# jerinphilip/whisper.tflite

Measured on AMD Instinct MI355X. Metric: audio-sec/s (RTF) whisper-tiny 30s clips batch=32 at 1/2/4/8 MI355X, higher is better.
Workload: dtype f32 (operands as two fp16 planes, f16 MFMA, f32 accumulate); 1 GPU; whisper-tiny batch=32x30s synthetic mel U(-1,1.5), fp32, random-init weights (BASELINE.json configs[1]); mel resident in HBM -> token ids on host; clips_per_gpu=32, global_batch=32, decoder_positions=30, argmax_steps=27, parallelism=clip-parallel dp1, one RCCL all_gather of id records per 8 batches, pipelined=True, batches_in_flight=10, decoder=2 consecutive steps' batches share one decoder chain (dec_pair, dec_group), last_batches_announced=2, priming_batches=1

## Files before the change

include/wt_debug.h:

```cpp
#ifndef WT_DEBUG_H_
#define WT_DEBUG_H_
#include "wt_capi.h"
#ifdef __cplusplus
extern "C" {
#endif
int wt_dbg_gemm(wt_engine* h, int M, int N, int K, const float* A, const float* W, const float* bias,
                const float* R, const float* pos, int pos_period, int epi, float* C);
int wt_dbg_gemm_planes(wt_engine* h, int M, int N, int K, const float* A, const float* W, const float* bias,
                       const float* R, const float* pos, int pos_period, int epi, int planes_out, int iters, float* C,
                       float* avg_ms, int n_cu );
int wt_dbg_set_forced_ids(wt_engine* h, const int64_t* ids, int clips);
int wt_dbg_set_plane_gemm_mode(int mode);
int wt_dbg_gemm_planes_ln(wt_engine* h, int M, int K, const float* A, const float* W, const float* bias, const float* R,
                          const float* pos, int pos_period, int epi, const float* ln_g, const float* ln_b, int n_cu,
                          float* C, float* ln_out, float* ln_y32, int* fused);
int wt_dbg_encoder_attention_planes(wt_engine* h, int batch, int T, int heads, const float* qkv, int iters, float* out,
                                    float* avg_ms);
int wt_dbg_gemm_bench(wt_engine* h, int M, int N, int K, int epi, int variant, int iters, float* avg_ms);
int wt_dbg_interference(wt_engine* h, const float* d_mel, int batch, int n_enc, int chain_len, int blocks,
                        float* enc_ms, float* chain_ms);
int wt_dbg_concurrency(wt_engine* h, const float* d_mel, int batch, int n_dec, int n_enc, float* dec_ms,
                       float* enc_ms);
int wt_dbg_dec_gemm_bench(wt_engine* h, int kind, int B, int N, int K, int rows, int iters, float* avg_us);
int wt_dbg_dec_gemm(wt_engine* h, int mode, int B, int N, int K, const float* X, const float* W,
// ... 35 lines not shown
                               float* kcache, float* vcache, float* out);
int wt_dbg_cross_attention_bf16(wt_engine* h, int batch, int heads, int T, int chunks, int nq, const float* x,
                                const float* ln_g, const float* ln_b, const float* wq, const float* bq, const float* kc,
                                const float* vc, float* out);
int wt_dbg_beam_topk(wt_engine* h, int rows, int V, int ldl, int kk, const float* logits, float* m, float* s,
                     uint64_t* keys);
int wt_dbg_beam_step(wt_engine* h, int K, int clips, int c0, int n_live, int pos, int n_prompt, int V, int64_t eot,
                     const float* logits, const int64_t* ids, float* live_sum, int32_t* fin_tok, float* fin_sum,
                     int32_t* fin_len, int32_t* n_fin, int32_t* done, int32_t* parent, int64_t* token, int64_t* ids_next);
int wt_dbg_beam_reorder(wt_engine* h, int src_rows, int dst_rows, int cap, int d, int slabs, int pos, int V,
                        const float* kv_src, float* kv_dst, const int64_t* ids_src, int64_t* ids_dst,
                        const int32_t* parent, const int64_t* token);
int wt_dbg_beam_finalize(wt_engine* h, int K, int clips, int c0, int pos, int n_prompt, const int64_t* ids,
                         const float* live_sum, int32_t* fin_tok, float* fin_sum, int32_t* fin_len, int32_t* n_fin,
                         const int32_t* done, int64_t* out_ids, int32_t* out_n, float* out_sum, int32_t* out_len);
int wt_dbg_dec_gemm_ksplit(wt_engine* h, int bf16, int M, int B, int N, int K, const float* X, const float* W,
                           const float* bias, float* R, float* Y, float* part);
int wt_dbg_dec_ln_gemm_rows(wt_engine* h, int bf16, int M, int B, int N, int K, const float* xin, const float* xpart,
                            const int64_t* ids, int ids_stride, int pos, const float* tok_emb, const float* pos_emb,
                            int n_vocab, int n_pos, const float* ln_g, const float* ln_b, const float* W, const float* bias,
                            int gelu, float* Y, float* xout);
int wt_dbg_dec_logits(wt_engine* h, int bf16, int M, int V, int K, const float* xin, const float* xpart, const float* ln_g,
                      const float* ln_b, const float* E, int blocks, float* logits, uint64_t* records);
int wt_dbg_select_token(wt_engine* h, int B, int n_tiles, const uint64_t* records, int64_t* ids, int stride, int pos,
                        int32_t* n_ids, int32_t* finished, int64_t eot, int stop_at_eot, int keep_ids);
int wt_dbg_language_head(wt_engine* h, int rows, int d, int n_vocab, int lang_lo, int n_lang, int forced_lang, const float* x,
                         const float* xpart, const float* ln_g, const float* ln_b, const float* tok_emb, float* probs,
                         int32_t* lang, float* lang_prob, int64_t* ids, int ids_stride);
#ifdef __cplusplus
}
#endif
#endif
```

whisper.tflite_amd/__init__.py:

```python
from __future__ import annotations

import ctypes
import enum
import os
from ctypes import (POINTER, byref, c_char_p, c_float, c_int, c_int32, c_int64, c_long, c_size_t,
                    c_uint64, c_void_p)

import numpy as np

_HERE = os.path.dirname(os.path.abspath(__file__))
LIB_PATH = os.environ.get("WT_LIB_PATH") or os.path.join(_HERE, "lib", "libwhisper-tflite.so")

WT_OK = 0
WT_MAX_IDS = 32
WT_PIPELINE_DEPTH = 24
WT_LANGUAGE_AUTO = -1
CHUNK_SAMPLES = 480000
STATUS_NAMES = {0: "WT_OK", 1: "WT_ERR_INVALID_ARG", 2: "WT_ERR_IO", 3: "WT_ERR_FORMAT",
                4: "WT_ERR_UNSUPPORTED", 5: "WT_ERR_DEVICE", 6: "WT_ERR_BUFFER"}

CAPI_SYMBOLS = [
    "wt_device_alloc", "wt_device_free", "wt_device_upload", "wt_device_download", "wt_device_synchronize",
    "wt_engine_create", "wt_engine_destroy", "wt_last_error", "wt_engine_dims",
    "wt_engine_set_option", "wt_engine_get_option", "wt_engine_set_prompt", "wt_transcribe_pcm", "wt_transcribe_long_pcm", "wt_transcribe_file",
    "wt_logmel_batch", "wt_logmel_batch_dev", "wt_encdec_tokens_batch",
    "wt_encdec_tokens_batch_dev", "wt_transcribe_tokens_batch_dev", "wt_pipeline_submit_dev", "wt_pipeline_submit_pcm_dev", "wt_pipeline_collect",
    "wt_encdec_debug_batch",
    "wt_encdec_tokens_full_batch", "wt_encdec_tokens_full_batch_dev", "wt_transcribe_tokens_full_batch_dev",
    "wt_language_count", "wt_detect_language_batch", "wt_detect_language_batch_dev", "wt_detect_language_pcm", "wt_last_languages",
    "wt_last_timings", "wt_last_beam_scores", "wt_last_kernel_stats", "wt_decode_text", "wt_language_id", "wt_lang_code", "wt_wav_read_legacy",
    "wt_vocab_info", "wt_filters", "wt_write_synthetic_weights", "wt_write_synthetic_vocab",
    "wt_vocab_open", "wt_vocab_close", "wt_vocab_get_info", "wt_vocab_get_filters", "wt_vocab_size", "wt_vocab_token",
    "wt_vocab_decode", "wt_log_mel_spectrogram", "wt_convert_tflite", "wt_shutdown",
]
DEBUG_SYMBOLS = [
    "wt_dbg_cross_absorbed", "wt_dbg_cross_absorbed_bf16", "wt_dbg_gemm_planes_ln", "wt_dbg_gemm", "wt_dbg_gemm_bench", "wt_dbg_dec_gemm_bench", "wt_dbg_dec_gemm", "wt_dbg_dec_ln_gemm", "wt_dbg_layernorm", "wt_dbg_encoder_attention",
    "wt_dbg_cross_attention", "wt_dbg_self_attention", "wt_dbg_interference", "wt_dbg_concurrency",
    "wt_dbg_gemm_planes", "wt_dbg_set_plane_gemm_mode", "wt_dbg_set_forced_ids", "wt_dbg_dec_gemm_bf16", "wt_dbg_dec_ln_gemm_bf16",
    "wt_dbg_self_attention_bf16", "wt_dbg_cross_attention_bf16", "wt_dbg_encoder_attention_planes", "wt_dbg_gemm_bf16", "wt_dbg_gemm_bf16_ln", "wt_dbg_encoder_attention_bf16",
    "wt_dbg_beam_topk", "wt_dbg_beam_step", "wt_dbg_beam_reorder", "wt_dbg_beam_finalize",
    "wt_dbg_dec_gemm_ksplit", "wt_dbg_dec_ln_gemm_rows", "wt_dbg_dec_logits", "wt_dbg_select_token",
    "wt_dbg_cross_absorbed_chain", "wt_dbg_absorbed_query_matrix", "wt_dbg_language_head", "wt_dbg_self_attention_long",
]


class WtError(RuntimeError):
    def __init__(self, code: int, message: str):
        super().__init__(f"{STATUS_NAMES.get(code, code)}: {message}")
        self.code = code


class EngineType(enum.IntEnum):
    Monolith = 0
    EncDec = 1


class Dims(ctypes.Structure):
    _fields_ = [(n, c_int32) for n in (
        "n_mels", "n_audio_ctx", "n_audio_state", "n_audio_head", "n_audio_layer",
        "n_vocab", "n_text_ctx", "n_text_state", "n_text_head", "n_text_layer")]


class Timings(ctypes.Structure):
    _fields_ = [("logmel_ms", c_float), ("encoder_ms", c_float), ("cross_kv_ms", c_float),
# ... 87 lines not shown
        L.wt_device_upload.argtypes = [c_void_p, c_void_p, ctypes.c_size_t, c_void_p, ctypes.c_size_t]
        L.wt_device_download.argtypes = [c_void_p, c_void_p, c_void_p, ctypes.c_size_t, ctypes.c_size_t]
        L.wt_device_synchronize.argtypes = [c_void_p]
        L.wt_dbg_set_forced_ids.argtypes = [c_void_p, POINTER(c_int64), c_int]
        L.wt_dbg_dec_gemm_bf16.argtypes = L.wt_dbg_dec_gemm.argtypes
        L.wt_dbg_dec_ln_gemm_bf16.argtypes = L.wt_dbg_dec_ln_gemm.argtypes
        L.wt_dbg_encoder_attention.argtypes = [c_void_p, c_int, c_int, c_int, fp, fp]
        L.wt_dbg_cross_attention.argtypes = [c_void_p, c_int, c_int, c_int, c_int, c_int, fp, fp, fp, fp, fp, fp, fp, fp]
        L.wt_dbg_self_attention.argtypes = [c_void_p, c_int, c_int, c_int, c_int, c_int, fp, fp, fp, fp]
        L.wt_dbg_self_attention_bf16.argtypes = L.wt_dbg_self_attention.argtypes
        L.wt_dbg_cross_attention_bf16.argtypes = L.wt_dbg_cross_attention.argtypes
        u64p = POINTER(c_uint64)
        L.wt_dbg_beam_topk.argtypes = [c_void_p, c_int, c_int, c_int, c_int, fp, fp, fp, u64p]
        L.wt_dbg_beam_step.argtypes = [c_void_p, c_int, c_int, c_int, c_int, c_int, c_int, c_int, c_int64, fp, ip64, fp, ip32,
                                       fp, ip32, ip32, ip32, ip32, ip64, ip64]
        L.wt_dbg_beam_reorder.argtypes = [c_void_p, c_int, c_int, c_int, c_int, c_int, c_int, c_int, fp, fp, ip64, ip64, ip32,
                                          ip64]
        L.wt_dbg_beam_finalize.argtypes = [c_void_p, c_int, c_int, c_int, c_int, c_int, ip64, fp, ip32, fp, ip32, ip32, ip32,
                                           ip64, ip32, fp, ip32]
        L.wt_dbg_dec_gemm_ksplit.argtypes = [c_void_p, c_int, c_int, c_int, c_int, c_int, fp, fp, fp, fp, fp, fp]
        L.wt_dbg_dec_ln_gemm_rows.argtypes = [c_void_p, c_int, c_int, c_int, c_int, c_int, fp, fp, ip64, c_int, c_int, fp, fp,
                                              c_int, c_int, fp, fp, fp, fp, c_int, fp, fp]
        L.wt_dbg_dec_logits.argtypes = [c_void_p, c_int, c_int, c_int, c_int, fp, fp, fp, fp, fp, c_int, fp, u64p]
        L.wt_dbg_select_token.argtypes = [c_void_p, c_int, c_int, u64p, ip64, c_int, c_int, ip32, ip32, c_int64, c_int,
                                          c_int]
        L.wt_language_count.argtypes = [c_void_p]
        L.wt_detect_language_batch.argtypes = [c_void_p, fp, c_int, ip32, fp]
        L.wt_detect_language_batch_dev.argtypes = [c_void_p, c_void_p, c_int, ip32, fp]
        L.wt_detect_language_pcm.argtypes = [c_void_p, fp, c_size_t, ip32, fp]
        L.wt_last_languages.argtypes = [c_void_p, ip32, fp, c_int]
        L.wt_dbg_language_head.argtypes = [c_void_p, c_int, c_int, c_int, c_int, c_int, c_int, fp, fp, fp, fp, fp, fp, ip32, fp,
                                           ip64, c_int]
        L.wt_encdec_tokens_full_batch.argtypes = [c_void_p, fp, c_int, ip64, c_int, ip32]
        L.wt_encdec_tokens_full_batch_dev.argtypes = [c_void_p, c_void_p, c_int, ip64, c_int, ip32]
        L.wt_transcribe_tokens_full_batch_dev.argtypes = [c_void_p, c_void_p, c_int, ip64, c_int, ip32]
        L.wt_dbg_self_attention_long.argtypes = [c_void_p, c_int, c_int, c_int, c_int, fp, fp, fp, fp]
        _lib = L
    return _lib


def _f32(a) -> np.ndarray:
    return np.ascontiguousarray(a, dtype=np.float32)


def _fp(a: np.ndarray):
    return a.ctypes.data_as(POINTER(c_float)) if a is not None else None
# ... 635 lines not shown
        N, K = W.shape
        xin = _f32(xin) if xin is not None else None
        xpart = _f32(xpart) if xpart is not None else None
        ids_a = np.ascontiguousarray(ids, dtype=np.int64) if ids is not None else None
        tok_emb = _f32(tok_emb) if tok_emb is not None else None
        pos_emb = _f32(pos_emb) if pos_emb is not None else None
        if ids_a is not None:
            B, stride = ids_a.shape
            M = M or B
        else:
            M, stride = xin.shape[0], 0
            B = B or M
        xout = np.array(xout, np.float32, order="C") if xout is not None else np.zeros((M + 1, K), np.float32)
        assert xout.shape == (M + 1, K)
        Y = np.zeros((M, N), np.float32)
        self._check(lib().wt_dbg_dec_ln_gemm_rows(
            self._h, int(bf16), M, B, N, K, _fp(xin), _fp(xpart), _ip64(ids_a) if ids_a is not None else None, stride, pos,
            _fp(tok_emb), _fp(pos_emb), tok_emb.shape[0] if tok_emb is not None else 0,
            pos_emb.shape[0] if pos_emb is not None else 0, _fp(ln_g), _fp(ln_b), _fp(W), _fp(bias), int(gelu), _fp(Y),
            _fp(xout)))
        return Y, xout

    def dbg_dec_logits(self, xin, ln_g, ln_b, E, xpart=None, blocks=0, bf16=False, want_logits=True,
                       logits_guard=1.0e30, records_guard=0xA5A5A5A5A5A5A5A5):
        xin, ln_g, ln_b, E = _f32(xin), _f32(ln_g), _f32(ln_b), _f32(E)
        xpart = _f32(xpart) if xpart is not None else None
        M, K = xin.shape
        V = E.shape[0]
        logits = np.full((M + 1, V), logits_guard, np.float32) if want_logits else None
        records = np.full((M + 1, (V + 31) // 32), records_guard, np.uint64)
        self._check(lib().wt_dbg_dec_logits(self._h, int(bf16), M, V, K, _fp(xin), _fp(xpart), _fp(ln_g), _fp(ln_b), _fp(E),
                                            blocks, _fp(logits), records.ctypes.data_as(POINTER(c_uint64))))
        return logits, records

    def dbg_language_head(self, x, ln_g, ln_b, tok_emb, lang_lo, n_lang, xpart=None, ids=None, forced_lang=-1):
        x, ln_g, ln_b, tok_emb = _f32(x), _f32(ln_g), _f32(ln_b), _f32(tok_emb)
        xpart = _f32(xpart) if xpart is not None else None
        rows, d = x.shape
        probs = np.full((rows, n_lang), np.nan, np.float32)
        lang = np.full(rows, -1, np.int32)
        prob = np.full(rows, np.nan, np.float32)
        ids = np.array(ids, np.int64, order="C") if ids is not None else None
        self._check(lib().wt_dbg_language_head(
            self._h, rows, d, tok_emb.shape[0], lang_lo, n_lang, forced_lang, _fp(x), _fp(xpart), _fp(ln_g), _fp(ln_b),
            _fp(tok_emb), _fp(probs), _ip32(lang), _fp(prob), _ip64(ids) if ids is not None else None,
            ids.shape[1] if ids is not None else 0))
        return probs, lang, prob, ids

    def dbg_select_token(self, records, ids, pos, n_ids, finished, eot, stop_at_eot=True, keep_ids=False):
        records = np.ascontiguousarray(records, dtype=np.uint64)
        B, n_tiles = records.shape
        ids = np.array(ids, np.int64, order="C")
        n_ids = np.array(n_ids, np.int32, order="C")
        finished = np.array(finished, np.int32, order="C")
        self._check(lib().wt_dbg_select_token(self._h, B, n_tiles, records.ctypes.data_as(POINTER(c_uint64)), _ip64(ids),
# ... 38 lines not shown
```

whisper.tflite_amd/csrc/capi.cpp:

```cpp
#include "wt_capi.h"

#include <hip/hip_runtime.h>

#include <functional>

#include <cstdio>
#include <cstdlib>
#include <sys/stat.h>
#include <unistd.h>
#include <cmath>
#include <cstring>
#include <memory>
#include <string>
#include <vector>

#include <mutex>

#include "engine.h"
#include "tflite_extract.h"
#include "weights_gen.h"
#include "wt_debug.h"
#include "kernels.h"

struct wt_engine {
// ... 1773 lines not shown
    const size_t mk = size_t(M) * K;
    DevArr<float> dxin(xin ? mk : 0, xin), dxp(xpart ? mk : 0, xpart);
    DevArr<long long> dids(ids ? size_t(B) * ids_stride : 0, reinterpret_cast<const long long*>(ids));
    DevArr<float> dtok(ids ? size_t(n_vocab) * K : 0, tok_emb), dpos(ids ? size_t(n_pos) * K : 0, pos_emb);
    DevArr<float> dg(K, ln_g), db(K, ln_b), dB(N, bias), dY(size_t(M) * N);
    DevArr<float> dxo(mk + K, xout);
    wt::DecGemmArgs g;
    g.bf16 = bf;
    g.Wt = dW.w(); g.w_scale = dW.scale; g.N = N; g.K = K; g.B = B; g.M = M;
    g.ln_g = dg.p; g.ln_b = db.p; g.xout = dxo.p;
    if (ids) {
      g.ids = dids.p; g.ids_stride = ids_stride; g.pos = pos; g.tok_emb = dtok.p; g.pos_emb = dpos.p; g.n_vocab = n_vocab;
    } else {
      g.xin = dxin.p; g.xpart = xpart ? dxp.p : nullptr;
    }
    g.bias = dB.p; g.Y = dY.p; g.ldy = N;
    wt::launch_dec_gemm(g, wt::kProLn, gelu ? wt::kDecBiasGelu : wt::kDecBias, h->impl->stream());
    h->impl->sync();
    dY.to_host(Y);
    dxo.to_host(xout);
  });
}

int wt_dbg_dec_logits(wt_engine* h, int bf16, int M, int V, int K, const float* xin, const float* xpart, const float* ln_g,
                      const float* ln_b, const float* E, int blocks, float* logits, uint64_t* records) {
  if (!h || !xin || !ln_g || !ln_b || !E || !records || M < 1 || M > 128 || V < 1 || blocks < 0 ||
      (K != 128 && K != 384 && K != 512)) {
    return WT_ERR_INVALID_ARG;
  }
  return guarded(h, [&] {
    const bool bf = bf16 != 0;
    const int n_tiles = (V + 31) / 32;
    const DevTiled dE(E, V, K, bf);
    const size_t mk = size_t(M) * K;
    DevArr<float> dxin(mk, xin), dxp(xpart ? mk : 0, xpart), dg(K, ln_g), db(K, ln_b);
    DevArr<float> dY(logits ? (size_t(M) + 1) * V : 0, logits);
    DevArr<unsigned long long> dBest((size_t(M) + 1) * n_tiles, reinterpret_cast<const unsigned long long*>(records));
    wt::DecGemmArgs g;
    g.bf16 = bf;
    g.logits_blocks = blocks;
    g.Wt = dE.w(); g.w_scale = dE.scale; g.N = V; g.K = K; g.B = M; g.M = M;
    g.xin = dxin.p; g.xpart = xpart ? dxp.p : nullptr; g.ln_g = dg.p; g.ln_b = db.p;
    g.Y = logits ? dY.p : nullptr; g.ldy = V; g.best = dBest.p;
    wt::launch_dec_gemm(g, wt::kProLn, wt::kDecLogits, h->impl->stream());
    h->impl->sync();
    if (logits) dY.to_host(logits);
    dBest.to_host(reinterpret_cast<unsigned long long*>(records));
  });
}

int wt_dbg_select_token(wt_engine* h, int B, int n_tiles, const uint64_t* records, int64_t* ids, int stride, int pos,
                        int32_t* n_ids, int32_t* finished, int64_t eot, int stop_at_eot, int keep_ids) {
  if (!h || !records || !ids || !n_ids || !finished || B < 1 || n_tiles < 1 || pos < 0 || pos + 1 >= stride) {
    return WT_ERR_INVALID_ARG;
  }
  return guarded(h, [&] {
    DevArr<unsigned long long> dRec(size_t(B) * n_tiles, reinterpret_cast<const unsigned long long*>(records));
    DevArr<long long> dids(size_t(B) * stride, reinterpret_cast<const long long*>(ids));
    DevArr<int> dn(B, n_ids), dfin(B, finished);
    wt::launch_select_token(dRec.p, n_tiles, dids.p, stride, pos, dn.p, dfin.p, eot, stop_at_eot, B, h->impl->stream(),
                            keep_ids != 0);
    h->impl->sync();
    dids.to_host(reinterpret_cast<long long*>(ids));
    dn.to_host(n_ids);
    dfin.to_host(finished);
  });
}

int wt_dbg_language_head(wt_engine* h, int rows, int d, int n_vocab, int lang_lo, int n_lang, int forced_lang, const float* x,
                         const float* xpart, const float* ln_g, const float* ln_b, const float* tok_emb, float* probs,
                         int32_t* lang, float* lang_prob, int64_t* ids, int ids_stride) {
// ... 106 lines not shown
```

whisper.tflite_amd/csrc/k_decoder.hip:

```cpp
#include <hip/hip_runtime.h>

#include <cstdlib>

#include "bf16_split.h"
#include "kernels.h"

namespace wt {
namespace {

using f32x16 = __attribute__((ext_vector_type(16))) float;
using f32x4 = __attribute__((ext_vector_type(4))) float;
using half8 = __attribute__((ext_vector_type(8))) _Float16;

__device__ __forceinline__ float gelu_erf(float x) {
  return 0.5f * x * (1.0f + erff(x * 0.70710678118654752440f));
}
__device__ __forceinline__ unsigned ordered_bits(float v) {
  v = v + 0.0f;
  const unsigned u = __float_as_uint(v);
  return (u & 0x80000000u) ? ~u : (u | 0x80000000u);
}
__device__ __forceinline__ int crow(int r, int h) { return (r & 3) + 8 * (r >> 2) + 4 * h; }

struct DecGemmDev {
// ... 309 lines not shown
      const int m = (g0 + t) * 32 + crow(r, lh);
      float v = sum + bias;
      if (EPI == kDecBias && g.gelu) v = gelu_erf(v);
      const bool ok = n_ok && m < M;
      if (EPI == kDecResid && khalf == 1) {
        if (ok) g.part[(long)m * g.ldy + n_epi] = sum;
        continue;
      }
      if (EPI == kDecResid && ok) v += r_pre[EPI == kDecResid ? j : 0];
      if (ok && g.Y) g.Y[(long)m * g.ldy + n_epi] = v;
      if (EPI == kDecLogits) {
        unsigned long long p = ok ? (((unsigned long long)ordered_bits(v) << 32) | (unsigned)n_epi) : 0ull;
#pragma unroll
        for (int off = 16; off >= 1; off >>= 1) {
          const unsigned long long o2 = __shfl_xor(p, off, 64);
          p = o2 > p ? o2 : p;
        }
        if (l31 == 0 && m < M) g.best[(long)m * g.best_stride + tile] = p;
      }
    }
  }
}

template <int KS, bool BF, int LNMODE>
__global__ __launch_bounds__(256, 2) void dec_logits_persistent(DecGemmDev g) {
  constexpr int KC = KS * 64, XLD = KC + 4;
  constexpr int kRed = 2 * 4 * 16 * 64, kXs = LNMODE >= 0 ? 32 * XLD : 0;
  __shared__ __attribute__((aligned(16))) float smem_l[kRed > kXs ? kRed : kXs];
  float (*red)[4][16][64] = reinterpret_cast<float (*)[4][16][64]>(smem_l);
  const int tid = threadIdx.x, lane = tid & 63, wid = tid >> 6;
  const int l31 = lane & 31, lh = lane >> 5;
  const int n_tiles = (g.N + 31) / 32, K = g.K, M = g.M;
  const int k0 = wid * (K >> 2);
  constexpr int WSTEP = BF ? 512 : 1024;
  const unsigned short* const wbase = g.Wt + (long)(k0 >> 4) * WSTEP + lane * 8;
  const long tile_stride = (long)(K >> 4) * WSTEP;
  int tile = blockIdx.x;
  u32x4_t wh[KS], wl[BF ? 1 : KS];
  {
    const unsigned short* wp = wbase + (long)(tile < n_tiles ? tile : n_tiles - 1) * tile_stride;
#pragma unroll
    for (int s = 0; s < KS; ++s) {
      wh[s] = *reinterpret_cast<const u32x4_t*>(wp + (long)s * WSTEP);
      if (!BF) wl[s] = *reinterpret_cast<const u32x4_t*>(wp + (long)s * WSTEP + 512);
    }
  }
  u32x4_t ah[KS], al[BF ? 1 : KS];
  float inv = 1.0f;
  const int m0 = blockIdx.y * 32;
  if (LNMODE >= 0) {
    constexpr int NF4 = 2 * KS;
    const int r8 = lane >> 3, sub = lane & 7, lrow = wid * 8 + r8, row = m0 + lrow;
    const RowSrc src{g.xin, g.xpart, nullptr, 0, 0, g.B, nullptr, nullptr, 0};
    f32x4 v[NF4], gg[NF4], bb[NF4];
#pragma unroll
    for (int j = 0; j < NF4; ++j) {
      gg[j] = *reinterpret_cast<const f32x4*>(g.ln_g + (sub + 8 * j) * 4);
      bb[j] = *reinterpret_cast<const f32x4*>(g.ln_b + (sub + 8 * j) * 4);
    }
    load_row<NF4, LNMODE < 0 ? 0 : LNMODE>(v, src, row < M ? row : M - 1, sub, K);
    float mean, rstd;
    row_stats<NF4>(v, K, &mean, &rstd);
#pragma unroll
    for (int j = 0; j < NF4; ++j) {
      const int c = (sub + 8 * j) * 4;
      f32x4 o;
#pragma unroll
      for (int e = 0; e < 4; ++e) o[e] = (v[j][e] - mean) * rstd * gg[j][e] + bb[j][e];
      *reinterpret_cast<f32x4*>(&smem_l[lrow * XLD + c]) = o;
    }
    __syncthreads();
  }
  {
    int row = m0 + l31;
    row = row < M ? row : M - 1;
    const float* xp = (LNMODE >= 0 ? smem_l + l31 * XLD : g.X + (long)row * g.ldx) + k0 + 8 * lh;
    float xa[KS][8];
#pragma unroll
    for (int s = 0; s < KS; ++s) {
      const f32x4 a = *reinterpret_cast<const f32x4*>(xp + 16 * s);
      const f32x4 b = *reinterpret_cast<const f32x4*>(xp + 16 * s + 4);
#pragma unroll
      for (int e = 0; e < 4; ++e) {
        xa[s][e] = a[e];
        xa[s][4 + e] = b[e];
      }
    }
    if (BF) {
#pragma unroll
      for (int s = 0; s < KS; ++s)
#pragma unroll
        for (int e = 0; e < 4; ++e) ah[s][e] = pack_bf16x2(xa[s][2 * e], xa[s][2 * e + 1]);
    } else {
      float mx = 0.0f;
#pragma unroll
      for (int s = 0; s < KS; ++s)
#pragma unroll
        for (int e = 0; e < 8; ++e) mx = fmaxf(mx, fabsf(xa[s][e]));
      mx = fmaxf(mx, __shfl_xor(mx, 32, 64));
      const unsigned ex = (__float_as_uint(mx) >> 23) & 0xFFu;
      const float sc = ex < 32u ? 1.0f : __uint_as_float((268u - ex) << 23);
      inv = ex < 32u ? 1.0f : __uint_as_float((ex - 14u) << 23);
#pragma unroll
      for (int s = 0; s < KS; ++s) {
        u32x4_t pl[3];
        split8_f16x2(xa[s], sc, pl);
        ah[s] = pl[0];
        al[s] = pl[1];
      }
    }
  }
  if (LNMODE >= 0) __syncthreads();
  float rscale[16];
#pragma unroll
  for (int r = 0; r < 16; ++r) rscale[r] = BF ? 1.0f : __shfl(inv, crow(r, lh), 64) * g.w_descale;

  for (int par = 0; tile < n_tiles; tile += gridDim.x, par ^= 1) {
    const int nt = tile + (int)gridDim.x < n_tiles ? tile + (int)gridDim.x : tile;
    const unsigned short* np = wbase + (long)nt * tile_stride;
    u32x4_t nwh[KS], nwl[BF ? 1 : KS];
#pragma unroll
    for (int s = 0; s < KS; ++s) {
      nwh[s] = *reinterpret_cast<const u32x4_t*>(np + (long)s * WSTEP);
      if (!BF) nwl[s] = *reinterpret_cast<const u32x4_t*>(np + (long)s * WSTEP + 512);
    }
    f32x16 part;
#pragma unroll
    for (int r = 0; r < 16; ++r) part[r] = 0.0f;
#pragma unroll
    for (int s = 0; s < KS; ++s) {
      if (BF) {
        using bf16x8 = __attribute__((ext_vector_type(8))) __bf16;
        part = __builtin_amdgcn_mfma_f32_32x32x16_bf16(__builtin_bit_cast(bf16x8, ah[s]), __builtin_bit_cast(bf16x8, wh[s]), part, 0, 0, 0);
      } else {
        const half8 a_h = __builtin_bit_cast(half8, ah[s]), a_l = __builtin_bit_cast(half8, al[BF ? 0 : s]);
        const half8 b_h = __builtin_bit_cast(half8, wh[s]), b_l = __builtin_bit_cast(half8, wl[BF ? 0 : s]);
        part = __builtin_amdgcn_mfma_f32_32x32x16_f16(a_h, b_l, part, 0, 0, 0);
        part = __builtin_amdgcn_mfma_f32_32x32x16_f16(a_l, b_h, part, 0, 0, 0);
        part = __builtin_amdgcn_mfma_f32_32x32x16_f16(a_h, b_h, part, 0, 0, 0);
      }
    }
#pragma unroll
    for (int r = 0; r < 16; ++r) red[par][wid][r][lane] = BF ? part[r] : 0.0f + part[r] * rscale[r];
    __syncthreads();
    {
      const int n_epi = tile * 32 + l31;
      const bool n_ok = n_epi < g.N;
#pragma unroll
      for (int rr = 0; rr < 4; ++rr) {
        const int r = wid * 4 + rr;
        float v = red[par][0][r][lane];
        v += red[par][1][r][lane];
        v += red[par][2][r][lane];
        v += red[par][3][r][lane];
        v += 0.0f;
        const int m = m0 + crow(r, lh);
        const bool ok = n_ok && m < M;
        if (ok && g.Y) g.Y[(long)m * g.ldy + n_epi] = v;
        const unsigned key = ok ? ordered_bits(v) : 0u;
        unsigned kmax = key;
#pragma unroll
        for (int off = 16; off >= 1; off >>= 1) {
          const unsigned o2 = __shfl_xor(kmax, off, 64);
          kmax = o2 > kmax ? o2 : kmax;
        }
        const unsigned long long hit = __ballot(ok && key == kmax);
        const unsigned half_hits = (unsigned)(hit >> (32 * lh));
        if (l31 == 0 && m < M) {
          const unsigned col = half_hits ? (unsigned)(tile * 32 + 31 - __clz(half_hits)) : 0u;
          g.best[(long)m * g.best_stride + tile] = half_hits ? (((unsigned long long)kmax << 32) | col) : 0ull;
        }
      }
    }
#pragma unroll
    for (int s = 0; s < KS; ++s) {
      wh[s] = nwh[s];
      if (!BF) wl[s] = nwl[s];
    }
  }
}

template <bool BF, int LNMODE>
bool launch_logits_persistent(const DecGemmDev& g, hipStream_t s, int blocks = 0) {
  if (g.K % 64 != 0 || g.ksplit != 1) return false;
  const int n_tiles = (g.N + 31) / 32, m_tiles = (g.M + 31) / 32;
  static const int forced = [] {
    const char* v = getenv("WT_LOGITS_BLOCKS");
    const int n = v ? atoi(v) : 0;
    return n >= 32 && n <= 1024 ? n : 0;
  }();
  const int total = forced ? forced : (blocks >= 32 && blocks <= 1024 ? blocks : 512);
  const int per = total / m_tiles;
  const dim3 grid(n_tiles < per ? n_tiles : per, m_tiles);
  switch (g.K / 64) {
    case 2: hipLaunchKernelGGL((dec_logits_persistent<2, BF, LNMODE>), grid, dim3(256), 0, s, g); return true;
    case 6: hipLaunchKernelGGL((dec_logits_persistent<6, BF, LNMODE>), grid, dim3(256), 0, s, g); return true;
    case 8: hipLaunchKernelGGL((dec_logits_persistent<8, BF, LNMODE>), grid, dim3(256), 0, s, g); return true;
    default: return false;
  }
}

template <int NF4, int LNMODE>
__global__ __launch_bounds__(256) void dec_finalize_ln(RowSrc src, const float* __restrict__ g,
                                                       const float* __restrict__ b,
                                                       float* __restrict__ y, int B, int K) {
  const int lane = threadIdx.x & 63, wid = threadIdx.x >> 6;
  const int r8 = lane >> 3, sub = lane & 7;
  const int row = blockIdx.x * 32 + wid * 8 + r8;
  if (row >= B) return;
  f32x4 v[NF4], gg[NF4], bb[NF4];
#pragma unroll
  for (int j = 0; j < NF4; ++j) {
    gg[j] = *reinterpret_cast<const f32x4*>(g + (sub + 8 * j) * 4);
    bb[j] = *reinterpret_cast<const f32x4*>(b + (sub + 8 * j) * 4);
  }
  load_row<NF4, LNMODE>(v, src, row, sub, K);
  float mean, rstd;
  row_stats<NF4>(v, K, &mean, &rstd);
#pragma unroll
  for (int j = 0; j < NF4; ++j) {
// ... 39 lines not shown
  if (two) {
    launch_steps<PRO, EPI, NF4, LNMODE, WAVES, CH, 2, BF>(g, s);
  } else {
    launch_steps<PRO, EPI, NF4, LNMODE, WAVES, CH, 1, BF>(g, s);
  }
}

template <int LNMODE, bool BF>
void launch_ln(const DecGemmDev& g, hipStream_t s) {
  switch (g.K) {
    case 128: launch_gt<kProLn, kDecBias, 4, LNMODE, 4, 1, BF>(g, s); break;
    case 384: launch_gt<kProLn, kDecBias, 12, LNMODE, 4, 1, BF>(g, s); break;
    case 512: launch_gt<kProLn, kDecBias, 16, LNMODE, 4, 1, BF>(g, s); break;
    default: throw Error(kErrFormat, "decoder kernels support d_model 128, 384 or 512");
  }
}

}

template <bool BF>
static void dispatch_dec_gemm(const DecGemmArgs& a, const DecGemmDev& g, int pro, int epi, hipStream_t s) {
  if (pro == kProLn && epi == kDecLogits) {
    if (a.ids || !a.xin || !a.ln_g || !a.ln_b) throw Error(kErrInvalidArg, "logits GEMM: LayerNorm rows come from xin (+ xpart)");
    const bool ok = a.xpart ? launch_logits_persistent<BF, 3>(g, s, a.logits_blocks) : launch_logits_persistent<BF, 0>(g, s, a.logits_blocks);
    if (!ok) throw Error(kErrInvalidArg, "logits GEMM with the LayerNorm prologue: K must be a multiple of 64");
    return;
  }
  if (pro == kProLn) {
    if (epi != kDecBias) throw Error(kErrInvalidArg, "decoder GEMM: the LayerNorm prologue pairs with the bias epilogue");
    if (a.ids) {
      if (a.xpart) throw Error(kErrInvalidArg, "decoder GEMM: embedding rows have no pending partial");
      launch_ln<2, BF>(g, s);
    } else if (a.xpart) {
      launch_ln<3, BF>(g, s);
    } else {
      launch_ln<0, BF>(g, s);
    }
    return;
  }
  const int key = pro * 8 + epi;
  switch (key) {
    case kProNone * 8 + kDecResid: launch_gt<kProNone, kDecResid, 0, 0, 8, 1, BF>(g, s); break;
    case kProNone * 8 + kDecBias: launch_gt<kProNone, kDecBias, 0, 0, 4, 1, BF>(g, s); break;
    case kProNone * 8 + kDecLogits:
      if (!launch_logits_persistent<BF, -1>(g, s, a.logits_blocks)) launch_gt<kProNone, kDecLogits, 0, 0, 4, 1, BF>(g, s);
      break;
    case kProCombine * 8 + kDecResid:
      switch (a.chunks) {
        case 1: launch_gt<kProCombine, kDecResid, 0, 0, 8, 1, BF>(g, s); break;
        case 2: launch_gt<kProCombine, kDecResid, 0, 0, 8, 2, BF>(g, s); break;
        case 4: launch_gt<kProCombine, kDecResid, 0, 0, 8, 4, BF>(g, s); break;
        case 8: launch_gt<kProCombine, kDecResid, 0, 0, 8, 8, BF>(g, s); break;
        default: throw Error(kErrInvalidArg, "cross_chunks must be 1, 2, 4 or 8");
      }
      break;
    default: throw Error(kErrInvalidArg, "unsupported decoder GEMM prologue / epilogue pair");
  }
}

void launch_dec_gemm(const DecGemmArgs& a, int pro, int epi, hipStream_t s) {
  const int gelu = epi == kDecBiasGelu ? 1 : 0;
  if (epi == kDecBiasGelu) epi = kDecBias;
  const int M = a.M > 0 ? a.M : a.B;
  const int ksplit = a.ksplit > 0 ? a.ksplit : 1;
  DecGemmDev g{a.Wt,      1.0f / a.w_scale, a.N,  a.K,       M,         a.B,     a.X,     a.ldx,   a.xin,  a.xout,
               a.ln_g,    a.ln_b,    a.ids,      a.ids_stride, a.pos,   a.tok_emb, a.pos_emb, a.n_vocab,
               a.cross_ws, a.heads,  a.chunks,   a.bias,    gelu,      a.R,     a.Y,     a.ldy,   a.best,
               a.best_stride > 0 ? a.best_stride : (a.N + 31) / 32, ksplit, a.part,  a.xpart, 0};
// ... 42 lines not shown
```

whisper.tflite_amd/csrc/kernels.h:

```cpp
#pragma once
#include <hip/hip_runtime.h>
#include <hip/hip_ext.h>

#include <cstdint>
#include <vector>

#include "error.h"

namespace wt {

struct LaunchTimer {
  hipEvent_t start = nullptr, stop = nullptr;
};
extern thread_local LaunchTimer g_launch_timer;

#define WT_LAUNCH_TIMED(kernel, grid, block, smem, stream, ...)                                                      \
  do {                                                                                                                \
    if (::wt::g_launch_timer.start) {                                                                                 \
      hipExtLaunchKernelGGL(kernel, grid, block, smem, stream, ::wt::g_launch_timer.start, ::wt::g_launch_timer.stop, \
                            0, __VA_ARGS__);                                                                          \
    } else {                                                                                                          \
      hipLaunchKernelGGL(kernel, grid, block, smem, stream, __VA_ARGS__);                                             \
    }                                                                                                                 \
  } while (0)
// ... 61 lines not shown
  float* ln_y32 = nullptr;
  int* nonfinite = nullptr;
};
bool launch_gemm_planes(const PlaneGemmArgs& a, int epi, hipStream_t s);
int plane_gemm_mode();
void set_plane_gemm_mode(int m);
bool launch_gemm_bf16_planes(const PlaneGemmArgs& a, int epi, hipStream_t s);
std::vector<unsigned short> round_weights_bf16(const float* W, int N, int K, int Kpad);
std::vector<unsigned short> split_weight_planes(const float* W, int N, int K, int Kpad, float scale);

enum DecPro : int {
  kProNone = 0,
  kProLn = 1,
  kProCombine = 2
};
enum DecEpi : int {
  kDecResid = 0,
  kDecBias = 1,
  kDecBiasGelu = 2,
  kDecLogits = 3
};
struct DecGemmArgs {
  int logits_blocks = 0;
  const unsigned short* Wt = nullptr;
  float w_scale = 1.0f;
  int N = 0, K = 0, B = 0;
  int M = 0;
  const float* X = nullptr;
  int ldx = 0;
  const float* xin = nullptr;
  float* xout = nullptr;
  const float* ln_g = nullptr;
  const float* ln_b = nullptr;
  const long long* ids = nullptr;
  int ids_stride = 0, pos = 0;
  const float* tok_emb = nullptr;
  const float* pos_emb = nullptr;
  int n_vocab = 0;
  const float* cross_ws = nullptr;
  int heads = 0, chunks = 0;
  const float* bias = nullptr;
  const float* R = nullptr;
  float* Y = nullptr;
  int ldy = 0;
  unsigned long long* best = nullptr;
  int best_stride = 0;
// ... 147 lines not shown
```

Before: 150,000 audio-sec/s.

## Process two row tiles per block in persistent logits GEMM to reuse weight loads

The persistent decoder logits kernel can now handle two 32-row M tiles per block, so each vocab weight tile loaded from memory feeds two MFMA row tiles instead of one. This halves weight streaming over the large embedding matrix when M is at least 64. A compile-time option to prefetch two tiles ahead is also added but defaults to one. In exchange the kernel uses more registers and shared memory, and launch bounds drop to one block per SIMD occupancy hint, which may reduce latency hiding.

```diff
diff --git a/include/wt_debug.h b/include/wt_debug.h
--- a/include/wt_debug.h
+++ b/include/wt_debug.h
@@ -81,6 +81,8 @@
                             int gelu, float* Y, float* xout);
 int wt_dbg_dec_logits(wt_engine* h, int bf16, int M, int V, int K, const float* xin, const float* xpart, const float* ln_g,
                       const float* ln_b, const float* E, int blocks, float* logits, uint64_t* records);
+int wt_dbg_dec_logits_ex(wt_engine* h, int bf16, int M, int V, int K, const float* xin, const float* xpart, const float* ln_g,
+                         const float* ln_b, const float* E, int blocks, int row_tiles, float* logits, uint64_t* records);
 int wt_dbg_select_token(wt_engine* h, int B, int n_tiles, const uint64_t* records, int64_t* ids, int stride, int pos,
                         int32_t* n_ids, int32_t* finished, int64_t eot, int stop_at_eot, int keep_ids);
 int wt_dbg_language_head(wt_engine* h, int rows, int d, int n_vocab, int lang_lo, int n_lang, int forced_lang, const float* x,
diff --git a/whisper.tflite_amd/__init__.py b/whisper.tflite_amd/__init__.py
--- a/whisper.tflite_amd/__init__.py
+++ b/whisper.tflite_amd/__init__.py
@@ -39,7 +39,7 @@
     "wt_dbg_gemm_planes", "wt_dbg_set_plane_gemm_mode", "wt_dbg_set_forced_ids", "wt_dbg_dec_gemm_bf16", "wt_dbg_dec_ln_gemm_bf16",
     "wt_dbg_self_attention_bf16", "wt_dbg_cross_attention_bf16", "wt_dbg_encoder_attention_planes", "wt_dbg_gemm_bf16", "wt_dbg_gemm_bf16_ln", "wt_dbg_encoder_attention_bf16",
     "wt_dbg_beam_topk", "wt_dbg_beam_step", "wt_dbg_beam_reorder", "wt_dbg_beam_finalize",
-    "wt_dbg_dec_gemm_ksplit", "wt_dbg_dec_ln_gemm_rows", "wt_dbg_dec_logits", "wt_dbg_select_token",
+    "wt_dbg_dec_gemm_ksplit", "wt_dbg_dec_ln_gemm_rows", "wt_dbg_dec_logits", "wt_dbg_dec_logits_ex", "wt_dbg_select_token",
     "wt_dbg_cross_absorbed_chain", "wt_dbg_absorbed_query_matrix", "wt_dbg_language_head", "wt_dbg_self_attention_long",
 ]
 
@@ -173,6 +173,7 @@
         L.wt_dbg_dec_ln_gemm_rows.argtypes = [c_void_p, c_int, c_int, c_int, c_int, c_int, fp, fp, ip64, c_int, c_int, fp, fp,
                                               c_int, c_int, fp, fp, fp, fp, c_int, fp, fp]
         L.wt_dbg_dec_logits.argtypes = [c_void_p, c_int, c_int, c_int, c_int, fp, fp, fp, fp, fp, c_int, fp, u64p]
+        L.wt_dbg_dec_logits_ex.argtypes = [c_void_p, c_int, c_int, c_int, c_int, fp, fp, fp, fp, fp, c_int, c_int, fp, u64p]
         L.wt_dbg_select_token.argtypes = [c_void_p, c_int, c_int, u64p, ip64, c_int, c_int, ip32, ip32, c_int64, c_int,
                                           c_int]
         L.wt_language_count.argtypes = [c_void_p]
@@ -854,15 +855,16 @@
         return Y, xout
 
     def dbg_dec_logits(self, xin, ln_g, ln_b, E, xpart=None, blocks=0, bf16=False, want_logits=True,
-                       logits_guard=1.0e30, records_guard=0xA5A5A5A5A5A5A5A5):
-        xin, ln_g, ln_b, E = _f32(xin), _f32(ln_g), _f32(ln_b), _f32(E)
+                       logits_guard=1.0e30, records_guard=0xA5A5A5A5A5A5A5A5, row_tiles=0):
+        xin, E = _f32(xin), _f32(E)
+        ln_g, ln_b = (_f32(ln_g), _f32(ln_b)) if ln_g is not None else (None, None)
         xpart = _f32(xpart) if xpart is not None else None
         M, K = xin.shape
         V = E.shape[0]
         logits = np.full((M + 1, V), logits_guard, np.float32) if want_logits else None
         records = np.full((M + 1, (V + 31) // 32), records_guard, np.uint64)
-        self._check(lib().wt_dbg_dec_logits(self._h, int(bf16), M, V, K, _fp(xin), _fp(xpart), _fp(ln_g), _fp(ln_b), _fp(E),
-                                            blocks, _fp(logits), records.ctypes.data_as(POINTER(c_uint64))))
+        self._check(lib().wt_dbg_dec_logits_ex(self._h, int(bf16), M, V, K, _fp(xin), _fp(xpart), _fp(ln_g), _fp(ln_b), _fp(E),
+                                               blocks, row_tiles, _fp(logits), records.ctypes.data_as(POINTER(c_uint64))))
         return logits, records
 
     def dbg_language_head(self, x, ln_g, ln_b, tok_emb, lang_lo, n_lang, xpart=None, ids=None, forced_lang=-1):
diff --git a/whisper.tflite_amd/csrc/capi.cpp b/whisper.tflite_amd/csrc/capi.cpp
--- a/whisper.tflite_amd/csrc/capi.cpp
+++ b/whisper.tflite_amd/csrc/capi.cpp
@@ -1819,10 +1819,11 @@
   });
 }
 
-int wt_dbg_dec_logits(wt_engine* h, int bf16, int M, int V, int K, const float* xin, const float* xpart, const float* ln_g,
-                      const float* ln_b, const float* E, int blocks, float* logits, uint64_t* records) {
-  if (!h || !xin || !ln_g || !ln_b || !E || !records || M < 1 || M > 128 || V < 1 || blocks < 0 ||
-      (K != 128 && K != 384 && K != 512)) {
+int wt_dbg_dec_logits_ex(wt_engine* h, int bf16, int M, int V, int K, const float* xin, const float* xpart, const float* ln_g,
+                         const float* ln_b, const float* E, int blocks, int row_tiles, float* logits, uint64_t* records) {
+  const bool ln = ln_g && ln_b;
+  if (!h || !xin || (!ln && (ln_g || ln_b || xpart)) || !E || !records || M < 1 || M > 128 || V < 1 || blocks < 0 ||
+      row_tiles < 0 || row_tiles > 1 || (K != 128 && K != 384 && K != 512)) {
     return WT_ERR_INVALID_ARG;
   }
   return guarded(h, [&] {
@@ -1830,20 +1831,31 @@
     const int n_tiles = (V + 31) / 32;
     const DevTiled dE(E, V, K, bf);
     const size_t mk = size_t(M) * K;
-    DevArr<float> dxin(mk, xin), dxp(xpart ? mk : 0, xpart), dg(K, ln_g), db(K, ln_b);
+    DevArr<float> dxin(mk, xin), dxp(xpart ? mk : 0, xpart), dg(ln ? K : 0, ln_g), db(ln ? K : 0, ln_b);
     DevArr<float> dY(logits ? (size_t(M) + 1) * V : 0, logits);
     DevArr<unsigned long long> dBest((size_t(M) + 1) * n_tiles, reinterpret_cast<const unsigned long long*>(records));
     wt::DecGemmArgs g;
     g.bf16 = bf;
     g.logits_blocks = blocks;
+    g.logits_row_tiles = row_tiles;
     g.Wt = dE.w(); g.w_scale = dE.scale; g.N = V; g.K = K; g.B = M; g.M = M;
-    g.xin = dxin.p; g.xpart = xpart ? dxp.p : nullptr; g.ln_g = dg.p; g.ln_b = db.p;
+    if (ln) {
+      g.xin = dxin.p; g.xpart = xpart ? dxp.p : nullptr; g.ln_g = dg.p; g.ln_b = db.p;
+    } else {
+      g.X = dxin.p; g.ldx = K;
+    }
     g.Y = logits ? dY.p : nullptr; g.ldy = V; g.best = dBest.p;
-    wt::launch_dec_gemm(g, wt::kProLn, wt::kDecLogits, h->impl->stream());
+    wt::launch_dec_gemm(g, ln ? wt::kProLn : wt::kProNone, wt::kDecLogits, h->impl->stream());
     h->impl->sync();
     if (logits) dY.to_host(logits);
     dBest.to_host(reinterpret_cast<unsigned long long*>(records));
   });
+}
+
+int wt_dbg_dec_logits(wt_engine* h, int bf16, int M, int V, int K, const float* xin, const float* xpart, const float* ln_g,
+                      const float* ln_b, const float* E, int blocks, float* logits, uint64_t* records) {
+  if (!ln_g || !ln_b) return WT_ERR_INVALID_ARG;
+  return wt_dbg_dec_logits_ex(h, bf16, M, V, K, xin, xpart, ln_g, ln_b, E, blocks, 0, logits, records);
 }
 
 int wt_dbg_select_token(wt_engine* h, int B, int n_tiles, const uint64_t* records, int64_t* ids, int stride, int pos,
diff --git a/whisper.tflite_amd/csrc/k_decoder.hip b/whisper.tflite_amd/csrc/k_decoder.hip
--- a/whisper.tflite_amd/csrc/k_decoder.hip
+++ b/whisper.tflite_amd/csrc/k_decoder.hip
@@ -355,57 +355,76 @@
   }
 }
 
-template <int KS, bool BF, int LNMODE>
-__global__ __launch_bounds__(256, 2) void dec_logits_persistent(DecGemmDev g) {
+#ifndef WT_LOGITS_PF
+#define WT_LOGITS_PF 1
+#endif
+template <int KS, bool BF, int LNMODE, int RT, int PF>
+__global__ __launch_bounds__(256, RT == 1 ? 2 : 1) void dec_logits_persistent(DecGemmDev g) {
+  static_assert((RT == 1 || RT == 2) && (PF == 1 || PF == 2), "one or two row tiles, one or two tiles ahead");
   constexpr int KC = KS * 64, XLD = KC + 4;
-  constexpr int kRed = 2 * 4 * 16 * 64, kXs = LNMODE >= 0 ? 32 * XLD : 0;
+  constexpr int kRed = 2 * RT * 4 * 16 * 64, kXs = LNMODE >= 0 ? 32 * XLD : 0;
   __shared__ __attribute__((aligned(16))) float smem_l[kRed > kXs ? kRed : kXs];
-  float (*red)[4][16][64] = reinterpret_cast<float (*)[4][16][64]>(smem_l);
+  float (*red)[RT][4][16][64] = reinterpret_cast<float (*)[RT][4][16][64]>(smem_l);
   const int tid = threadIdx.x, lane = tid & 63, wid = tid >> 6;
   const int l31 = lane & 31, lh = lane >> 5;
   const int n_tiles = (g.N + 31) / 32, K = g.K, M = g.M;
   const int k0 = wid * (K >> 2);
+  const int gx = (int)gridDim.x;
   constexpr int WSTEP = BF ? 512 : 1024;
   const unsigned short* const wbase = g.Wt + (long)(k0 >> 4) * WSTEP + lane * 8;
   const long tile_stride = (long)(K >> 4) * WSTEP;
+  using wset = u32x4_t[KS];
+  using wset_lo = u32x4_t[BF ? 1 : KS];
+  auto load_w = [&](wset& h, wset_lo& l, int t) {
+    const unsigned short* wp = wbase + (long)t * tile_stride;
+#pragma unroll
+    for (int s = 0; s < KS; ++s) {
+      h[s] = *reinterpret_cast<const u32x4_t*>(wp + (long)s * WSTEP);
+      if (!BF) l[s] = *reinterpret_cast<const u32x4_t*>(wp + (long)s * WSTEP + 512);
+    }
+  };
   int tile = blockIdx.x;
-  u32x4_t wh[KS], wl[BF ? 1 : KS];
-  {
-    const unsigned short* wp = wbase + (long)(tile < n_tiles ? tile : n_tiles - 1) * tile_stride;
-#pragma unroll
-    for (int s = 0; s < KS; ++s) {
-      wh[s] = *reinterpret_cast<const u32x4_t*>(wp + (long)s * WSTEP);
-      if (!BF) wl[s] = *reinterpret_cast<const u32x4_t*>(wp + (long)s * WSTEP + 512);
-    }
-  }
-  u32x4_t ah[KS], al[BF ? 1 : KS];
-  float inv = 1.0f;
-  const int m0 = blockIdx.y * 32;
+  wset wh, nwh, fwh;
+  wset_lo wl, nwl, fwl;
+  load_w(wh, wl, tile < n_tiles ? tile : n_tiles - 1);
+  if (PF == 2) load_w(nwh, nwl, tile + gx < n_tiles ? tile + gx : (tile < n_tiles ? tile : n_tiles - 1));
+  u32x4_t ah[RT][KS], al[RT][BF ? 1 : KS];
+  float inv[RT];
+  const int m0 = blockIdx.y * (RT * 32);
+  const bool two = RT == 2 && m0 + 32 < M;
+  constexpr int NF4 = LNMODE >= 0 ? 2 * KS : 1;
+  f32x4 v[RT][NF4], gg[NF4], bb[NF4];
+  const int r8 = lane >> 3, sub = lane & 7, lrow = wid * 8 + r8;
   if (LNMODE >= 0) {
-    constexpr int NF4 = 2 * KS;
-    const int r8 = lane >> 3, sub = lane & 7, lrow = wid * 8 + r8, row = m0 + lrow;
     const RowSrc src{g.xin, g.xpart, nullptr, 0, 0, g.B, nullptr, nullptr, 0};
-    f32x4 v[NF4], gg[NF4], bb[NF4];
 #pragma unroll
     for (int j = 0; j < NF4; ++j) {
       gg[j] = *reinterpret_cast<const f32x4*>(g.ln_g + (sub + 8 * j) * 4);
       bb[j] = *reinterpret_cast<const f32x4*>(g.ln_b + (sub + 8 * j) * 4);
     }
-    load_row<NF4, LNMODE < 0 ? 0 : LNMODE>(v, src, row < M ? row : M - 1, sub, K);
-    float mean, rstd;
-    row_stats<NF4>(v, K, &mean, &rstd);
-#pragma unroll
-    for (int j = 0; j < NF4; ++j) {
-      const int c = (sub + 8 * j) * 4;
-      f32x4 o;
-#pragma unroll
-      for (int e = 0; e < 4; ++e) o[e] = (v[j][e] - mean) * rstd * gg[j][e] + bb[j][e];
-      *reinterpret_cast<f32x4*>(&smem_l[lrow * XLD + c]) = o;
-    }
-    __syncthreads();
-  }
-  {
-    int row = m0 + l31;
+#pragma unroll
+    for (int t = 0; t < RT; ++t) {
+      const int row = m0 + 32 * t + lrow;
+      load_row<NF4, LNMODE < 0 ? 0 : LNMODE>(v[t], src, row < M ? row : M - 1, sub, K);
+    }
+  }
+#pragma unroll
+  for (int t = 0; t < RT; ++t) {
+    if (LNMODE >= 0) {
+      if (t > 0) __syncthreads();
+      float mean, rstd;
+      row_stats<NF4>(v[t], K, &mean, &rstd);
+#pragma unroll
+      for (int j = 0; j < NF4; ++j) {
+        const int c = (sub + 8 * j) * 4;
+        f32x4 o;
+#pragma unroll
+        for (int e = 0; e < 4; ++e) o[e] = (v[t][j][e] - mean) * rstd * gg[j][e] + bb[j][e];
+        *reinterpret_cast<f32x4*>(&smem_l[lrow * XLD + c]) = o;
+      }
+      __syncthreads();
+    }
+    int row = m0 + 32 * t + l31;
     row = row < M ? row : M - 1;
     const float* xp = (LNMODE >= 0 ? smem_l + l31 * XLD : g.X + (long)row * g.ldx) + k0 + 8 * lh;
     float xa[KS][8];
@@ -419,11 +438,12 @@
         xa[s][4 + e] = b[e];
       }
     }
+    inv[t] = 1.0f;
     if (BF) {
 #pragma unroll
       for (int s = 0; s < KS; ++s)
 #pragma unroll
-        for (int e = 0; e < 4; ++e) ah[s][e] = pack_bf16x2(xa[s][2 * e], xa[s][2 * e + 1]);
+        for (int e = 0; e < 4; ++e) ah[t][s][e] = pack_bf16x2(xa[s][2 * e], xa[s][2 * e + 1]);
     } else {
       float mx = 0.0f;
 #pragma unroll
@@ -433,61 +453,67 @@
       mx = fmaxf(mx, __shfl_xor(mx, 32, 64));
       const unsigned ex = (__float_as_uint(mx) >> 23) & 0xFFu;
       const float sc = ex < 32u ? 1.0f : __uint_as_float((268u - ex) << 23);
-      inv = ex < 32u ? 1.0f : __uint_as_float((ex - 14u) << 23);
+      inv[t] = ex < 32u ? 1.0f : __uint_as_float((ex - 14u) << 23);
 #pragma unroll
       for (int s = 0; s < KS; ++s) {
         u32x4_t pl[3];
         split8_f16x2(xa[s], sc, pl);
-        ah[s] = pl[0];
-        al[s] = pl[1];
+        ah[t][s] = pl[0];
+        al[t][BF ? 0 : s] = pl[1];
       }
     }
   }
   if (LNMODE >= 0) __syncthreads();
-  float rscale[16];
-#pragma unroll
-  for (int r = 0; r < 16; ++r) rscale[r] = BF ? 1.0f : __shfl(inv, crow(r, lh), 64) * g.w_descale;
-
-  for (int par = 0; tile < n_tiles; tile += gridDim.x, par ^= 1) {
-    const int nt = tile + (int)gridDim.x < n_tiles ? tile + (int)gridDim.x : tile;
-    const unsigned short* np = wbase + (long)nt * tile_stride;
-    u32x4_t nwh[KS], nwl[BF ? 1 : KS];
+  float rscale[RT][16];
+#pragma unroll
+  for (int t = 0; t < RT; ++t)
+#pragma unroll
+    for (int r = 0; r < 16; ++r) rscale[t][r] = BF ? 1.0f : __shfl(inv[t], crow(r, lh), 64) * g.w_descale;
+
+  auto item = [&](const wset& ch, const wset_lo& cl, wset& fh, wset_lo& fl, int tile, int par) {
+    int ft = tile + gx < n_tiles ? tile + gx : tile;
+    if (PF == 2) ft = tile + 2 * gx < n_tiles ? tile + 2 * gx : ft;
+    load_w(fh, fl, ft);
+    f32x16 part[RT];
+#pragma unroll
+    for (int t = 0; t < RT; ++t)
+#pragma unroll
+      for (int r = 0; r < 16; ++r) part[t][r] = 0.0f;
 #pragma unroll
     for (int s = 0; s < KS; ++s) {
-      nwh[s] = *reinterpret_cast<const u32x4_t*>(np + (long)s * WSTEP);
-      if (!BF) nwl[s] = *reinterpret_cast<const u32x4_t*>(np + (long)s * WSTEP + 512);
-    }
-    f32x16 part;
-#pragma unroll
-    for (int r = 0; r < 16; ++r) part[r] = 0.0f;
-#pragma unroll
-    for (int s = 0; s < KS; ++s) {
-      if (BF) {
-        using bf16x8 = __attribute__((ext_vector_type(8))) __bf16;
-        part = __builtin_amdgcn_mfma_f32_32x32x16_bf16(__builtin_bit_cast(bf16x8, ah[s]), __builtin_bit_cast(bf16x8, wh[s]), part, 0, 0, 0);
-      } else {
-        const half8 a_h = __builtin_bit_cast(half8, ah[s]), a_l = __builtin_bit_cast(half8, al[BF ? 0 : s]);
-        const half8 b_h = __builtin_bit_cast(half8, wh[s]), b_l = __builtin_bit_cast(half8, wl[BF ? 0 : s]);
-        part = __builtin_amdgcn_mfma_f32_32x32x16_f16(a_h, b_l, part, 0, 0, 0);
-        part = __builtin_amdgcn_mfma_f32_32x32x16_f16(a_l, b_h, part, 0, 0, 0);
-        part = __builtin_amdgcn_mfma_f32_32x32x16_f16(a_h, b_h, part, 0, 0, 0);
-      }
-    }
-#pragma unroll
-    for (int r = 0; r < 16; ++r) red[par][wid][r][lane] = BF ? part[r] : 0.0f + part[r] * rscale[r];
+#pragma unroll
+      for (int t = 0; t < RT; ++t) {
+        if (BF) {
+          using bf16x8 = __attribute__((ext_vector_type(8))) __bf16;
+          part[t] = __builtin_amdgcn_mfma_f32_32x32x16_bf16(__builtin_bit_cast(bf16x8, ah[t][s]), __builtin_bit_cast(bf16x8, ch[s]), part[t], 0, 0, 0);
+        } else {
+          const half8 a_h = __builtin_bit_cast(half8, ah[t][s]), a_l = __builtin_bit_cast(half8, al[t][BF ? 0 : s]);
+          const half8 b_h = __builtin_bit_cast(half8, ch[s]), b_l = __builtin_bit_cast(half8, cl[BF ? 0 : s]);
+          part[t] = __builtin_amdgcn_mfma_f32_32x32x16_f16(a_h, b_l, part[t], 0, 0, 0);
+          part[t] = __builtin_amdgcn_mfma_f32_32x32x16_f16(a_l, b_h, part[t], 0, 0, 0);
+          part[t] = __builtin_amdgcn_mfma_f32_32x32x16_f16(a_h, b_h, part[t], 0, 0, 0);
+        }
+      }
+    }
+#pragma unroll
+    for (int t = 0; t < RT; ++t)
+#pragma unroll
+      for (int r = 0; r < 16; ++r) red[par][t][wid][r][lane] = BF ? part[t][r] : 0.0f + part[t][r] * rscale[t][r];
     __syncthreads();
-    {
-      const int n_epi = tile * 32 + l31;
-      const bool n_ok = n_epi < g.N;
+    const int n_epi = tile * 32 + l31;
+    const bool n_ok = n_epi < g.N;
+#pragma unroll
+    for (int t = 0; t < RT; ++t) {
+      if (t > 0 && !two) continue;
 #pragma unroll
       for (int rr = 0; rr < 4; ++rr) {
         const int r = wid * 4 + rr;
-        float v = red[par][0][r][lane];
-        v += red[par][1][r][lane];
-        v += red[par][2][r][lane];
-        v += red[par][3][r][lane];
+        float v = red[par][t][0][r][lane];
+        v += red[par][t][1][r][lane];
+        v += red[par][t][2][r][lane];
+        v += red[par][t][3][r][lane];
         v += 0.0f;
-        const int m = m0 + crow(r, lh);
+        const int m = m0 + 32 * t + crow(r, lh);
         const bool ok = n_ok && m < M;
         if (ok && g.Y) g.Y[(long)m * g.ldy + n_epi] = v;
         const unsigned key = ok ? ordered_bits(v) : 0u;
@@ -505,16 +531,34 @@
         }
       }
     }
-#pragma unroll
-    for (int s = 0; s < KS; ++s) {
-      wh[s] = nwh[s];
-      if (!BF) wl[s] = nwl[s];
+  };
+
+  if (PF == 1) {
+    for (int par = 0; tile < n_tiles; tile += gx, par ^= 1) {
+      item(wh, wl, nwh, nwl, tile, par);
+#pragma unroll
+      for (int s = 0; s < KS; ++s) {
+        wh[s] = nwh[s];
+        if (!BF) wl[s] = nwl[s];
+      }
+    }
+  } else if (tile < n_tiles) {
+    for (int par = 0;;) {
+      item(wh, wl, fwh, fwl, tile, par);
+      tile += gx, par ^= 1;
+      if (tile >= n_tiles) break;
+      item(nwh, nwl, wh, wl, tile, par);
+      tile += gx, par ^= 1;
+      if (tile >= n_tiles) break;
+      item(fwh, fwl, nwh, nwl, tile, par);
+      tile += gx, par ^= 1;
+      if (tile >= n_tiles) break;
     }
   }
 }
 
 template <bool BF, int LNMODE>
-bool launch_logits_persistent(const DecGemmDev& g, hipStream_t s, int blocks = 0) {
+bool launch_logits_persistent(const DecGemmDev& g, hipStream_t s, int blocks = 0, int row_tiles = 0) {
   if (g.K % 64 != 0 || g.ksplit != 1) return false;
   const int n_tiles = (g.N + 31) / 32, m_tiles = (g.M + 31) / 32;
   static const int forced = [] {
@@ -523,12 +567,23 @@
     return n >= 32 && n <= 1024 ? n : 0;
   }();
   const int total = forced ? forced : (blocks >= 32 && blocks <= 1024 ? blocks : 512);
-  const int per = total / m_tiles;
-  const dim3 grid(n_tiles < per ? n_tiles : per, m_tiles);
+  const bool rt2 = m_tiles >= 2 && row_tiles != 1;
+  const int m_groups = rt2 ? (m_tiles + 1) / 2 : m_tiles;
+  const int per = total / m_groups;
+  const dim3 grid(n_tiles < per ? n_tiles : per, m_groups);
+  constexpr int PF = WT_LOGITS_PF;
+  if (rt2) {
+    switch (g.K / 64) {
+      case 2: hipLaunchKernelGGL((dec_logits_persistent<2, BF, LNMODE, 2, PF>), grid, dim3(256), 0, s, g); return true;
+      case 6: hipLaunchKernelGGL((dec_logits_persistent<6, BF, LNMODE, 2, PF>), grid, dim3(256), 0, s, g); return true;
+      case 8: hipLaunchKernelGGL((dec_logits_persistent<8, BF, LNMODE, 2, PF>), grid, dim3(256), 0, s, g); return true;
+      default: return false;
+    }
+  }
   switch (g.K / 64) {
-    case 2: hipLaunchKernelGGL((dec_logits_persistent<2, BF, LNMODE>), grid, dim3(256), 0, s, g); return true;
-    case 6: hipLaunchKernelGGL((dec_logits_persistent<6, BF, LNMODE>), grid, dim3(256), 0, s, g); return true;
-    case 8: hipLaunchKernelGGL((dec_logits_persistent<8, BF, LNMODE>), grid, dim3(256), 0, s, g); return true;
+    case 2: hipLaunchKernelGGL((dec_logits_persistent<2, BF, LNMODE, 1, 1>), grid, dim3(256), 0, s, g); return true;
+    case 6: hipLaunchKernelGGL((dec_logits_persistent<6, BF, LNMODE, 1, 1>), grid, dim3(256), 0, s, g); return true;
+    case 8: hipLaunchKernelGGL((dec_logits_persistent<8, BF, LNMODE, 1, 1>), grid, dim3(256), 0, s, g); return true;
     default: return false;
   }
 }
@@ -614,7 +669,8 @@
 static void dispatch_dec_gemm(const DecGemmArgs& a, const DecGemmDev& g, int pro, int epi, hipStream_t s) {
   if (pro == kProLn && epi == kDecLogits) {
     if (a.ids || !a.xin || !a.ln_g || !a.ln_b) throw Error(kErrInvalidArg, "logits GEMM: LayerNorm rows come from xin (+ xpart)");
-    const bool ok = a.xpart ? launch_logits_persistent<BF, 3>(g, s, a.logits_blocks) : launch_logits_persistent<BF, 0>(g, s, a.logits_blocks);
+    const bool ok = a.xpart ? launch_logits_persistent<BF, 3>(g, s, a.logits_blocks, a.logits_row_tiles)
+                            : launch_logits_persistent<BF, 0>(g, s, a.logits_blocks, a.logits_row_tiles);
     if (!ok) throw Error(kErrInvalidArg, "logits GEMM with the LayerNorm prologue: K must be a multiple of 64");
     return;
   }
@@ -635,7 +691,7 @@
     case kProNone * 8 + kDecResid: launch_gt<kProNone, kDecResid, 0, 0, 8, 1, BF>(g, s); break;
     case kProNone * 8 + kDecBias: launch_gt<kProNone, kDecBias, 0, 0, 4, 1, BF>(g, s); break;
     case kProNone * 8 + kDecLogits:
-      if (!launch_logits_persistent<BF, -1>(g, s, a.logits_blocks)) launch_gt<kProNone, kDecLogits, 0, 0, 4, 1, BF>(g, s);
+      if (!launch_logits_persistent<BF, -1>(g, s, a.logits_blocks, a.logits_row_tiles)) launch_gt<kProNone, kDecLogits, 0, 0, 4, 1, BF>(g, s);
       break;
     case kProCombine * 8 + kDecResid:
       switch (a.chunks) {
diff --git a/whisper.tflite_amd/csrc/kernels.h b/whisper.tflite_amd/csrc/kernels.h
--- a/whisper.tflite_amd/csrc/kernels.h
+++ b/whisper.tflite_amd/csrc/kernels.h
@@ -107,6 +107,7 @@
 };
 struct DecGemmArgs {
   int logits_blocks = 0;
+  int logits_row_tiles = 0;
   const unsigned short* Wt = nullptr;
   float w_scale = 1.0f;
   int N = 0, K = 0, B = 0;
```

After: 148,600 audio-sec/s. About the same (-1.0%).
